# google/neural-light-transport

Measured on AMD Instinct MI355X. Metric: rendered Mtexels/s at 1024^2 UV (full Model.call forward: U-Net + UV->camera warp); at N > 1: N collective-free replicas of this forward (weak scaling).  The data-parallel TRAIN step with the RCCL gradient all-reduce (BASELINE config 4) is `train_step`: value = Mtexels/s over all ranks, speedup_vs_o, higher is better.
Workload: dtype f32 via 3xbf16 split, 9 exact products, fp32 accumulate (the LDS-tiled encoder convs: fp32 operands as three bf16 terms on v_mfma_f32_16x16x32_bf16, every term product exact in fp32); f32 storage everywhere, every other launch native f32; 1 GPU; BASELINE config 3: dragon_specular relight+view-synth, depth0 16/depth 256, 4 frames/GPU, 1024^2 UV, k=4 obs maps, 512^2 camera warp; frames_per_gpu=4, uv=1024, k=4, cam=512, conv_algo=auto, plan=fused ends, launch=eager, two HIP streams, distinct_batches_rotated=3, launch_tape_replays=0, parallelism=dp1 (frames sharded, no forward collective), world=1, dist_world_size=1, device=cuda:0

## Files before the change

include/nlt_hip.h:

```cpp
#ifndef NLT_HIP_H_
#define NLT_HIP_H_

#ifdef __cplusplus
extern "C" {
#endif

typedef enum {
  NLT_OK = 0,
  NLT_ERR_BAD_ARG = -1,
  NLT_ERR_UNSUPPORTED = -2,
  NLT_ERR_LAUNCH = -3
} nlt_status;

typedef enum {
  NLT_CONV1X1 = 0,
  NLT_CONV_K2S2 = 1,
  NLT_CONV_K2S1 = 2,
  NLT_DECONV_K2S2 = 3,
  NLT_DECONV_K2S1 = 4,
  NLT_CONV_K3S1 = 5,
  NLT_CONV_K3S2 = 6,
  NLT_DECONV_K3S1 = 7,
  NLT_DECONV_K3S2 = 8
} nlt_conv_mode;
// ... 351 lines not shown
                          const float* p2, int add_base, float alpha, float* q1, int ldq, float* skip3,
                          float* qtmp2, void* stream);
int nlt_front_ovr_forward_u8(const unsigned char* diffuse_store, const unsigned char* cvis_store,
                             const unsigned char* lvis_store, const int* ids, int n, int h, int w,
                             const float* packed, const float* packed_l2, const float* p1, const float* s0,
                             const float* p2, int add_base, float alpha, float* q1, int ldq, float* skip3,
                             float* qtmp2, void* stream);

int nlt_conv_backward_data(int adj_mode, int tile_hint, int ksplit, float* workspace,
                           const float* dpre, int ldp, int cpre, int n, int h, int w,
                           const float* w_packed, const float* zero_bias, int cout, float* out, int ldo,
                           const float* mask_src, int ldm, float mask_alpha, int accumulate,
                           int split_c, const float* split_y, float* split_d, float split_alpha, int split_partial,
                           void* stream);

long nlt_conv_wino_packed_floats(int mode, int cin, int cout, int tn);
int nlt_pack_conv_wino_weights(int mode, const float* w_keras, int cin, int cout, int tn, float* packed, void* stream);
int nlt_conv_wino_forward(int mode, const float* src, int ld, int cin, int frames, int kobs, int h, int w,
                          const float* packed, const float* bias, int cout, int tn,
                          float* out, int ldo, float* mean_out, int ldm, int act, float alpha, void* stream);
int nlt_pack_conv_wino_weights_adjoint(int adj_mode, const float* w_keras, int cpre, int cout, int tn, int full, int lo,
                                       float* packed, void* stream);
int nlt_conv_wino_backward_data(int adj_mode, const float* dpre, int ldp, int cpre, int n, int h, int w,
                                const float* packed, int cout, int tn, float* out, int ldo,
                                const float* mask_src, int ldm, float mask_alpha, int accumulate, void* stream);

int nlt_conv_c32_supported(int mode, int cin, int cout);
int nlt_conv_c32_forward(int mode, const float* src, int ld, int cin, int frames, int kobs, int h, int w,
                         const float* packed, const float* bias, int cout,
                         float* out, int ldo, float* mean_out, int ldm, int act, float alpha, void* stream);

long nlt_conv_tile_packed_floats(int mode, int cin, int cout, int tn);
int nlt_pack_conv_tile_weights(int mode, const float* w_keras, int cin, int cout, int tn, float* packed, void* stream);
int nlt_conv_tile_forward(int mode, const float* src, int ld, int cin, int frames, int kobs, int h, int w,
                          const float* packed, const float* bias, int cout, int tn,
                          float* out, int ldo, float* mean_out, int ldm, int act, float alpha, void* stream);

int nlt_pack_conv_tile_weights_adjoint(int adj_mode, const float* w_keras, int cpre, int cout, int tn, int full, int lo,
                                       float* packed, void* stream);
int nlt_conv_tile_backward_data(int adj_mode, const float* dpre, int ldp, int cpre, int n, int h, int w,
                                const float* packed, int cout, int tn, float* out, int ldo,
                                const float* mask_src, int ldm, float mask_alpha, int accumulate,
                                int split_c, const float* split_y, float* split_d, float split_alpha, int split_partial,
                                void* stream);

long nlt_conv_tile3_packed_elems(int mode, int cin, int cout, int tn);
int nlt_pack_conv_tile3_weights(int mode, const float* w_keras, int cin, int cout, int tn, unsigned short* packed, void* stream);
int nlt_conv_tile3_forward(int mode, int nprod, const float* src, int ld, int cin, int frames, int kobs, int h, int w,
                           const unsigned short* packed, const float* bias, int cout, int tn,
                           float* out, int ldo, float* mean_out, int ldm, int act, float alpha, void* stream);
int nlt_conv_tile3r_forward(int mode, int nprod, const float* src, int ld, int cin, int frames, int kobs, int h, int w,
                            const unsigned short* packed, const float* bias, int cout, int tn,
                            float* out, int ldo, float* mean_out, int ldm, int act, float alpha, int max_workgroups, void* stream);
long nlt_conv_tile3w_s2_packed_elems(int cin2, int cout2);
int nlt_pack_conv_tile3w_s2_weights(const float* w_keras, int cin2, int cout2, unsigned short* packed, void* stream);
long nlt_conv_tile3w_s2_lds_bytes(int cin, int cout, int cout2);
int nlt_conv_tile3w_s2_forward(int nprod, const float* src, int ld, int cin, int frames, int kobs, int h, int w,
                               const unsigned short* packed, const float* bias, int cout, float* out, int ldo,
                               float* mean_out, int ldm, int act, float alpha,
                               const unsigned short* packed2, const float* bias2, int cout2, float* out2, int ldo2,
                               int act2, float alpha2, int max_workgroups, void* stream);

long nlt_chmix_bf16_packed_elems(int cin, int cout);
int nlt_chmix_bf16_pack(const float* w_keras, int cin, int cout, unsigned short* packed, void* stream);
int nlt_chmix_bf16_forward(const unsigned short* x, long texels, int cin, const unsigned short* packed,
                           const float* bias, int cout, int act, float alpha, unsigned short* out, void* stream);

int nlt_conv_k3_forward(int mode, int algo, const float* x, int n, int h, int w, int cin,
                        const float* w_keras, const float* bias, int cout, float* y,
                        int act, float alpha, void* stream);

int nlt_conv_k3_backward_data(int mode, int algo, const float* dpre, int n, int h, int w, int cin,
                              const float* w_keras, int cout, float* dx, void* stream);

long nlt_conv_k3_wgrad_workspace_floats(int mode, int n, int h, int w, int cin, int cout);
int nlt_conv_k3_backward_weights(int mode, const float* x, int n, int h, int w, int cin,
                                 const float* dpre, int cout, float* dw_keras, float* dbias,
                                 float* workspace, long workspace_floats, void* stream);

#ifdef __cplusplus
}
#endif
#endif
```

neural-light-transport_amd/_capi.py:

```python
import ctypes
import threading
import os

import torch

_HERE = os.path.dirname(os.path.abspath(__file__))
LIB_PATH = os.environ.get('NLT_HIP_LIB') or os.path.join(_HERE, 'libnlt_hip.so')

CONV1X1, CONV_K2S2, CONV_K2S1, DECONV_K2S2, DECONV_K2S1 = range(5)
CONV_K3S1, CONV_K3S2, DECONV_K3S1, DECONV_K3S2 = range(5, 9)
ALGO_AUTO, ALGO_DIRECT, ALGO_MFMA = range(3)

_c_int, _c_long, _c_float, _vp = ctypes.c_int, ctypes.c_long, ctypes.c_float, ctypes.c_void_p
_c_double = ctypes.c_double
MAP_F64, MAP_F32, MAP_F16 = range(3)

SIGNATURES = {
    'nlt_version': (ctypes.c_char_p, []),
    'nlt_status_string': (ctypes.c_char_p, [_c_int]),
    'nlt_packed_weight_floats': (_c_long, [_c_int] * 4),
    'nlt_pack_conv_weights': (_c_int, [_c_int, _vp, _c_int, _c_int, _c_int, _vp, _vp]),
    'nlt_conv_forward': (_c_int, [_c_int, _c_int, _c_int, _vp, _c_int, _c_int, _vp, _c_int, _c_int,
                                  _c_int, _c_int, _c_int, _vp, _vp, _vp, _c_int, _vp, _c_int,
                                  _c_int, _c_float, _vp, _c_int, _c_int, _vp]),
# ... 56 lines not shown
    'nlt_front_packed_floats': (_c_long, []),
    'nlt_front_pack_weights': (_c_int, [_vp] * 15 + [_vp]),
    'nlt_front_forward': (_c_int, [_vp] * 5 + [_c_int] * 4 + [_vp, _c_int, _c_float, _vp, _vp, _vp, _vp]),
    'nlt_front_l2_packed_floats': (_c_long, []),
    'nlt_front_pack_l2_weights': (_c_int, [_vp] * 5 + [_vp]),
    'nlt_front2_forward': (_c_int, [_vp] * 5 + [_c_int] * 4 + [_vp, _vp, _c_int, _c_float, _vp, _vp, _vp, _vp, _vp]),
    'nlt_front4_forward': (_c_int, [_vp] * 5 + [_c_int] * 4 + [_vp, _vp, _c_int, _c_float, _vp, _vp, _vp, _vp, _c_int, _vp]),
    'nlt_front4_forward_u8': (_c_int, [_vp] * 6 + [_c_int] * 4 + [_vp, _vp, _c_int, _c_float, _vp, _vp, _vp, _vp, _c_int, _vp]),
    'nlt_front4_forward_train': (_c_int, [_vp] * 5 + [_c_int] * 4 + [_vp, _vp, _c_int, _c_float] + [_vp] * 7 + [_vp]),
    'nlt_dec_block_forward': (_c_int, [_vp, _c_int, _vp, _c_int, _c_int, _c_int, _c_int, _vp, _vp, _vp, _vp, _c_int, _c_float, _vp, _vp]),
    'nlt_back_forward': (_c_int, [_vp] * 3 + [_c_int] * 3 + [_vp] * 5 + [_c_float, _vp, _vp]),
    'nlt_front_forward_train': (_c_int, [_vp] * 5 + [_c_int] * 4 + [_vp, _c_int, _c_float] + [_vp] * 6),
    'nlt_back_forward_train': (_c_int, [_vp] * 3 + [_c_int] * 3 + [_vp] * 5 + [_c_float] + [_vp] * 4),
    'nlt_front_backward_workspace_floats': (_c_long, [_c_int] * 3),
    'nlt_front_backward': (_c_int, [_vp] * 5 + [_c_int] * 4 + [_vp] * 21),
    'nlt_back_backward_workspace_floats': (_c_long, [_c_int] * 3),
    'nlt_back_backward': (_c_int, [_vp] * 5 + [_c_int] * 3 + [_vp] * 3 + [_c_float] + [_vp] * 10),
    'nlt_conv_splitk_workspace_floats': (_c_long, [_c_int] * 6),
    'nlt_conv_forward_splitk': (_c_int, [_c_int, _c_int, _c_int, _vp, _vp, _c_int, _c_int, _vp, _c_int, _c_int,
                                         _c_int, _c_int, _c_int, _vp, _vp, _c_int, _vp, _c_int, _c_int, _c_float,
                                         _vp, _c_int, _c_int, _vp]),
    'nlt_conv_forward_map': (_c_int, [_c_int, _c_int, _c_int, _vp, _vp, _c_int, _c_int, _vp, _c_int, _c_int,
                                      _c_int, _c_int, _c_int, _vp, _vp, _c_int, _vp, _c_int, _c_int, _c_float,
                                      _vp, _c_int, _vp]),
    'nlt_dec_block_forward_map': (_c_int, [_vp, _vp, _c_int, _c_int, _c_int, _c_int, _vp, _vp, _vp, _c_int, _c_float, _vp, _vp, _vp]),
    'nlt_back_forward_map': (_c_int, [_vp, _vp, _c_int, _vp, _c_int, _c_int, _c_int, _vp, _vp, _vp, _vp, _c_float, _vp, _vp, _vp]),
    'nlt_front_ovr_forward': (_c_int, [_vp] * 3 + [_c_int] * 3 + [_vp] * 5 + [_c_int, _c_float, _vp, _c_int, _vp, _vp, _vp]),
    'nlt_front_ovr_forward_u8': (_c_int, [_vp] * 4 + [_c_int] * 3 + [_vp] * 5 + [_c_int, _c_float, _vp, _c_int, _vp, _vp, _vp]),
    'nlt_conv_backward_data': (_c_int, [_c_int, _c_int, _c_int, _vp, _vp, _c_int, _c_int, _c_int, _c_int, _c_int, _vp, _vp, _c_int,
                                        _vp, _c_int, _vp, _c_int, _c_float, _c_int, _c_int, _vp, _vp, _c_float, _c_int, _vp]),
    'nlt_conv_tile_packed_floats': (_c_long, [_c_int] * 4),
    'nlt_pack_conv_tile_weights': (_c_int, [_c_int, _vp, _c_int, _c_int, _c_int, _vp, _vp]),
    'nlt_conv_tile_forward': (_c_int, [_c_int, _vp, _c_int, _c_int, _c_int, _c_int, _c_int, _c_int, _vp, _vp, _c_int, _c_int,
                                       _vp, _c_int, _vp, _c_int, _c_int, _c_float, _vp]),
    'nlt_pack_conv_tile_weights_adjoint': (_c_int, [_c_int, _vp, _c_int, _c_int, _c_int, _c_int, _c_int, _vp, _vp]),
    'nlt_conv_c32_supported': (_c_int, [_c_int] * 3),
    'nlt_conv_c32_forward': (_c_int, [_c_int, _vp, _c_int, _c_int, _c_int, _c_int, _c_int, _c_int, _vp, _vp, _c_int,
                                      _vp, _c_int, _vp, _c_int, _c_int, _c_float, _vp]),
    'nlt_conv_wino_packed_floats': (_c_long, [_c_int] * 4),
    'nlt_pack_conv_wino_weights': (_c_int, [_c_int, _vp, _c_int, _c_int, _c_int, _vp, _vp]),
    'nlt_conv_wino_forward': (_c_int, [_c_int, _vp, _c_int, _c_int, _c_int, _c_int, _c_int, _c_int, _vp, _vp, _c_int, _c_int,
                                       _vp, _c_int, _vp, _c_int, _c_int, _c_float, _vp]),
    'nlt_pack_conv_wino_weights_adjoint': (_c_int, [_c_int, _vp, _c_int, _c_int, _c_int, _c_int, _c_int, _vp, _vp]),
    'nlt_conv_wino_backward_data': (_c_int, [_c_int, _vp, _c_int, _c_int, _c_int, _c_int, _c_int, _vp, _c_int, _c_int, _vp, _c_int,
                                             _vp, _c_int, _c_float, _c_int, _vp]),
    'nlt_conv_tile_backward_data': (_c_int, [_c_int, _vp, _c_int, _c_int, _c_int, _c_int, _c_int, _vp, _c_int, _c_int, _vp, _c_int,
                                             _vp, _c_int, _c_float, _c_int, _c_int, _vp, _vp, _c_float, _c_int, _vp]),
    'nlt_conv_tile3_packed_elems': (_c_long, [_c_int] * 4),
    'nlt_pack_conv_tile3_weights': (_c_int, [_c_int, _vp, _c_int, _c_int, _c_int, _vp, _vp]),
    'nlt_conv_tile3_forward': (_c_int, [_c_int, _c_int, _vp, _c_int, _c_int, _c_int, _c_int, _c_int, _c_int, _vp, _vp, _c_int, _c_int,
                                        _vp, _c_int, _vp, _c_int, _c_int, _c_float, _vp]),
    'nlt_conv_tile3r_forward': (_c_int, [_c_int, _c_int, _vp, _c_int, _c_int, _c_int, _c_int, _c_int, _c_int, _vp, _vp, _c_int, _c_int,
                                         _vp, _c_int, _vp, _c_int, _c_int, _c_float, _c_int, _vp]),
    'nlt_conv_tile3w_s2_packed_elems': (_c_long, [_c_int] * 2),
    'nlt_pack_conv_tile3w_s2_weights': (_c_int, [_vp, _c_int, _c_int, _vp, _vp]),
    'nlt_conv_tile3w_s2_lds_bytes': (_c_long, [_c_int] * 3),
    'nlt_conv_tile3w_s2_forward': (_c_int, [_c_int, _vp, _c_int, _c_int, _c_int, _c_int, _c_int, _c_int, _vp, _vp, _c_int, _vp, _c_int,
                                            _vp, _c_int, _c_int, _c_float, _vp, _vp, _c_int, _vp, _c_int, _c_int, _c_float, _c_int, _vp]),
    'nlt_conv_bf16_packed_elems': (_c_long, [_c_int] * 4),
    'nlt_conv_bf16_pack': (_c_int, [_c_int, _vp, _c_int, _c_int, _c_int, _vp, _vp]),
    'nlt_conv_bf16_forward': (_c_int, [_c_int, _c_int, _vp, _c_int, _c_int, _c_int, _vp, _c_int, _c_int, _c_int,
                                       _c_int, _c_int, _c_int, _vp, _vp, _c_int, _vp, _c_int, _c_int, _c_int, _c_float, _vp]),
    'nlt_conv_bf16_forward_map': (_c_int, [_c_int, _c_int, _vp, _c_int, _c_int, _c_int, _vp, _c_int, _c_int, _c_int,
                                           _c_int, _c_int, _c_int, _vp, _vp, _c_int, _vp, _c_int, _c_int, _c_int, _c_float,
                                           _vp, _c_int, _vp]),
    'nlt_obs_mean_bf16': (_c_int, [_vp, _c_int, _c_int, _c_long, _c_int, _vp, _c_int, _vp]),
    'nlt_chmix_bf16_packed_elems': (_c_long, [_c_int, _c_int]),
    'nlt_chmix_bf16_pack': (_c_int, [_vp, _c_int, _c_int, _vp, _vp]),
    'nlt_chmix_bf16_forward': (_c_int, [_vp, _c_long, _c_int, _vp, _vp, _c_int, _c_int, _c_float, _vp, _vp]),
    'nlt_cosine_map': (_c_int, [_vp] * 4 + [_c_double] * 3 + [_c_long, _vp, _vp, _vp]),
    'nlt_albedo': (_c_int, [_vp, _c_int, _c_long, _vp, _vp, _vp]),
    'nlt_diffuse_base': (_c_int, [_vp, _vp, _c_int, _c_long, _vp, _vp]),
    'nlt_remap_bilinear_u8': (_c_int, [_vp, _c_int, _c_int, _c_int, _vp, _c_int, _c_int, _c_int, _c_int, _c_int, _vp, _vp]),
    'nlt_remap_bilinear_f32': (_c_int, [_vp, _c_int, _c_int, _c_int, _vp, _c_int, _c_int, _c_int, _c_int, _c_int, _vp, _vp]),
    'nlt_uv_index_map_workspace_bytes': (_c_long, [_c_int, _c_int, _c_long]),
    'nlt_uv_index_map': (_c_int, [_vp, _vp, _c_long, _c_int, _c_int, _c_int, _c_int, _c_double, _vp, _vp, _vp, _vp]),
    'nlt_knn_indices': (_c_int, [_vp, _c_int, _vp, _c_int, _c_int, _vp, _vp]),
    'nlt_psnr_sums': (_c_int, [_vp, _vp, _vp, _c_long, _c_int, _vp, _vp, _vp]),
    'nlt_gather_frames_u8': (_c_int, [_vp, _vp, _c_int, _c_long, _vp, _vp]),
    'nlt_assemble_batch': (_c_int, [_vp] * 6 + [_c_int, _c_int, _c_long, _c_int] + [_vp] * 6 + [_vp]),
    'nlt_warp_backward_det_workspace_bytes': (_c_long, [_c_int] * 5),
    'nlt_warp_backward_det': (_c_int, [_vp, _vp] + [_c_int] * 5 + [_vp, _vp, _c_long, _vp]),
    'nlt_resize_bilinear_backward_gather': (_c_int, [_vp] + [_c_int] * 6 + [_vp, _vp]),
    'nlt_loss_det_workspace_floats': (_c_long, [_c_int]),
    'nlt_l2_loss_forward_det': (_c_int, [_vp, _vp, _c_int, _c_long, _vp, _vp, _c_long, _vp]),
    'nlt_l2_loss_weighted_forward_det': (_c_int, [_vp, _vp, _vp, _c_int, _c_long, _c_int, _vp, _vp, _c_long, _vp]),
    'nlt_l2_train_loss_det': (_c_int, [_vp, _vp, _vp, _c_int, _c_long, _c_float, _vp, _vp, _vp, _vp, _c_long, _vp]),
    'nlt_barron_det_slots_floats': (_c_long, [_c_int] * 3),
    'nlt_barron_loss_det': (_c_int, [_vp, _vp, _c_int, _c_int, _c_int, _vp, _vp, _vp, _vp, _c_long, _vp]),
    'nlt_stem_backward_det_workspace_floats': (_c_long, [_c_int] * 4),
    'nlt_stem_backward_det': (_c_int, [_vp] * 6 + [_c_int] * 5 + [_vp] * 6 + [_vp, _c_long, _vp]),
    'nlt_head_backward_det_workspace_floats': (_c_long, [_c_int] * 5),
    'nlt_head_backward_det': (_c_int, [_vp, _c_int, _c_int, _vp, _c_int, _c_int, _vp, _vp, _c_int, _c_int, _c_int,
                                       _vp, _c_int, _vp, _c_int, _vp, _vp, _vp, _c_long, _vp]),
    'nlt_conv_backward_weights_det_workspace_floats': (_c_long, [_c_int] * 7),
    'nlt_conv_backward_weights_det': (_c_int, [_c_int, _c_int, _vp, _c_int, _c_int, _vp, _c_int, _c_int,
                                               _c_int, _c_int, _c_int, _vp, _c_int, _c_int, _vp, _vp, _vp, _c_long, _vp]),
    'nlt_conv_k3_forward': (_c_int, [_c_int, _c_int, _vp, _c_int, _c_int, _c_int, _c_int, _vp, _vp, _c_int, _vp, _c_int, _c_float, _vp]),
    'nlt_conv_k3_backward_data': (_c_int, [_c_int, _c_int, _vp, _c_int, _c_int, _c_int, _c_int, _vp, _c_int, _vp, _vp]),
    'nlt_conv_k3_wgrad_workspace_floats': (_c_long, [_c_int] * 6),
    'nlt_conv_k3_backward_weights': (_c_int, [_c_int, _vp, _c_int, _c_int, _c_int, _c_int, _vp, _c_int, _vp, _vp, _vp, _c_long, _vp]),
}

_real = None


# ... 808 lines not shown


def pack_conv_wino_weights(mode, w_keras, cin, cout, tn, full=None, lo=0):
    src = (mode, _ptr(_dense(w_keras, 'w_keras')), cin, cout, tn)
    if full is None:
        name, args = 'nlt_pack_conv_wino_weights', src
    else:
        name, args = 'nlt_pack_conv_wino_weights_adjoint', src + (full, lo)
    return _pack('nlt_conv_wino_packed_floats', (mode, cin, cout, tn), name, args, torch.float32, w_keras.device)


def conv_wino_forward(mode, src, ld, cin, frames, kobs, h, w, packed, bias, cout, tn, out, ldo, mean_out, ldm, act=True, alpha=0.3):
    _call('nlt_conv_wino_forward', mode, _ptr(src), ld, cin, frames, kobs, h, w, _ptr(packed), _ptr(bias), cout, tn, _ptr(out), ldo,
          _ptr(mean_out), ldm, 1 if act else 0, float(alpha))


def conv_wino_backward_data(adj_mode, dpre, cpre, ldp, n, h, w, packed, cout, tn, out, ldo, mask_src=None, ldm=0, mask_alpha=0.3,
                            accumulate=False):
    _call('nlt_conv_wino_backward_data', adj_mode, _ptr(dpre), ldp, cpre, n, h, w, _ptr(packed), cout, tn, _ptr(out), ldo,
          _ptr(mask_src), ldm, float(mask_alpha), 1 if accumulate else 0)


def pack_conv_tile3_weights(mode, w_keras, cin, cout, tn):
    return _pack('nlt_conv_tile3_packed_elems', (mode, cin, cout, tn),
                 'nlt_pack_conv_tile3_weights', (mode, _ptr(_dense(w_keras, 'w_keras')), cin, cout, tn), torch.int16, w_keras.device)


def conv_tile3_forward(mode, src, ld, cin, frames, kobs, h, w, packed, bias, cout, tn, out, ldo, mean_out, ldm,
                       act=True, alpha=0.3, nprod=6):
    _call('nlt_conv_tile3_forward', mode, nprod, _ptr(src), ld, cin, frames, kobs, h, w, packed.data_ptr(), _ptr(bias), cout, tn,
          _ptr(out), ldo, _ptr(mean_out), ldm, 1 if act else 0, float(alpha))


def conv_tile3r_plan(mode, cin, tn):
    if mode not in (CONV_K2S1, CONV_K2S2) or cin % 16 or tn not in (32, 64):
        return None
    if mode == CONV_K2S1 and tn == 32:
        for rows in (4, 2):
            lds = cin * 768 + 8 * 6 * (((rows + 1) * 17 + 15) // 16 * 16) * 16
            if lds <= 160 * 1024:
                return (lds, 8, 1, rows)
    lds = cin * (tn // 16) * 384 + 2 * 6 * (160 if mode == CONV_K2S1 else 272) * 16
    if lds > 160 * 1024:
        return None
    return (lds, 8, 1, 8) if 2 * lds > 160 * 1024 else (lds, 4, 2, 8)


def conv_tile3r_forward(mode, src, ld, cin, frames, kobs, h, w, packed, bias, cout, tn, out, ldo, mean_out, ldm,
                        act=True, alpha=0.3, nprod=6, max_workgroups=0):
    _call('nlt_conv_tile3r_forward', mode, nprod, _ptr(src), ld, cin, frames, kobs, h, w, packed.data_ptr(), _ptr(bias), cout, tn,
          _ptr(out), ldo, _ptr(mean_out), ldm, 1 if act else 0, float(alpha), max_workgroups)


def pack_conv_tile3w_s2_weights(w_keras, cin2, cout2):
    return _pack('nlt_conv_tile3w_s2_packed_elems', (cin2, cout2),
                 'nlt_pack_conv_tile3w_s2_weights', (_ptr(_dense(w_keras, 'w_keras')), cin2, cout2), torch.int16, w_keras.device)


def conv_tile3w_s2_plan(cin, cout, cout2):
    n = lib().nlt_conv_tile3w_s2_lds_bytes(cin, cout, cout2)
    return n if n > 0 else None


def conv_tile3w_s2_forward(src, ld, cin, frames, kobs, h, w, packed, bias, cout, mean_out, ldm, packed2, bias2, cout2, out2, ldo2,
                           act=True, alpha=0.3, act2=True, alpha2=0.3, nprod=6, max_workgroups=0, out=None, ldo=0):
    _call('nlt_conv_tile3w_s2_forward', nprod, _ptr(src), ld, cin, frames, kobs, h, w, packed.data_ptr(), _ptr(bias), cout,
          _ptr(out), ldo, _ptr(mean_out), ldm, 1 if act else 0, float(alpha), packed2.data_ptr(), _ptr(bias2), cout2,
          _ptr(out2), ldo2, 1 if act2 else 0, float(alpha2), max_workgroups)


def conv_bf16_pack(mode, w_keras, c0, c1, cout):
    return _pack('nlt_conv_bf16_packed_elems', (mode, c0, c1, cout),
                 'nlt_conv_bf16_pack', (mode, _ptr(_dense(w_keras, 'w_keras')), c0, c1, cout), torch.bfloat16, w_keras.device)


def _any_ptr(t, what):
    if t is None:
        return None, 0
    if not (t.is_cuda and t.dtype in (torch.float32, torch.bfloat16)):
        raise NLTError("%s: expected a float32 / bfloat16 CUDA tensor, got %s on %s" % (what, t.dtype, t.device))
    return t.data_ptr(), 1 if t.dtype == torch.float32 else 0


def conv_bf16_forward(mode, src0, c0, ld0, src1, c1, ld1, n, h, w, w_packed, bias, cout, out, ldo, act=True, alpha=0.3, tile_hint=0):
    p0, f0 = _any_ptr(src0, 'src0')
    p1, f1 = _any_ptr(src1, 'src1')
    po, fo = _any_ptr(out, 'out')
    _call('nlt_conv_bf16_forward', mode, tile_hint, p0, ld0, c0, f0, p1, ld1, c1, f1, n, h, w,
          _tptr(w_packed, torch.bfloat16, 'w_packed'), _ptr(bias), cout, po, ldo, fo, 1 if act else 0, float(alpha))


def conv_bf16_forward_map(mode, src0, c0, ld0, src1, c1, ld1, n, h, w, w_packed, bias, cout, out, ldo, bias_map,
                          act=True, alpha=0.3, tile_hint=0):
    p0, f0 = _any_ptr(src0, 'src0')
    p1, f1 = _any_ptr(src1, 'src1')
    po, fo = _any_ptr(out, 'out')
    _call('nlt_conv_bf16_forward_map', mode, tile_hint, p0, ld0, c0, f0, p1, ld1, c1, f1, n, h, w,
          _tptr(w_packed, torch.bfloat16, 'w_packed'), _ptr(bias), cout, po, ldo, fo, 1 if act else 0, float(alpha),
          _tptr(bias_map, torch.float32, 'bias_map'), bias_map.shape[0])


def obs_mean_bf16(obs, n, k, hw, c, out, ldo):
    if obs.dtype != torch.bfloat16 or out.dtype != torch.bfloat16:
        raise NLTError("obs_mean_bf16: bfloat16 tensors expected")
    _call('nlt_obs_mean_bf16', obs.data_ptr(), n, k, hw, c, out.data_ptr(), ldo)

# ... 252 lines not shown
```

neural-light-transport_amd/csrc/conv_tile3.hip:

```cpp
#include "nlt_common.h"
#include "pack_common.h"

namespace {

typedef __attribute__((ext_vector_type(8))) __bf16 bf16x8;
typedef unsigned short u16;
typedef unsigned int u32x4 __attribute__((ext_vector_type(4)));

constexpr int TH = 8, TW = 16;
constexpr int QS2 = 272, ODD2 = 132;
constexpr int PL = 160;

template <int MODE> struct T3;
template <> struct T3<NLT_CONV_K2S1> { static constexpr int PAIRS = 2, B_UNITS = 153 * 2, B_SLOTS = 6 * PL; };
template <> struct T3<NLT_CONV_K2S2> { static constexpr int PAIRS = 1, B_UNITS = 256 * 2, B_SLOTS = 6 * QS2; };

struct Tile3P {
  const float* src; const u16* packed; const float* bias;
  float* out; float* mean_out;
  int ld, cin, frames, kobs, h, w;
  int oh, ow, cout, ldo, ldm;
  int tiles_y, tiles_x, ncc;
  int act; float alpha;
};
// ... 241 lines not shown
  };
  auto store_b = [&](int buf) {
    u32x4* base = lds + 2 * A_SLOTS + buf * TT::B_SLOTS;
#pragma unroll
    for (int n = 0; n < NB; ++n)
      if (b_st[n]) split_store_unit(base + b_lds[n], BPL, rb[n][0], rb[n][1]);
  };

  f32x4 acc[KO][RT][CT], mean[RT][CT];
#pragma unroll
  for (int rt = 0; rt < RT; ++rt)
#pragma unroll
    for (int ct = 0; ct < CT; ++ct) {
      mean[rt][ct] = (f32x4){0.f, 0.f, 0.f, 0.f};
#pragma unroll
      for (int io = 0; io < KO; ++io) acc[io][rt][ct] = mean[rt][ct];
    }

  load_a(0);
  load_b(0, 0);
  store_a(0);
  store_b(0);
  __syncthreads();
  int q = 0;
  for (int gi = 0; gi < groups; ++gi) {
    for (int s = 0; s < spf; ++s) {
      const int sa = (gi * spf + s) & 1;
#pragma unroll
      for (int io = 0; io < KO; ++io, ++q) {
        const bool more = q + 1 < total;
        const bool new_slab = io + 1 == KO;
        int ns = s, ngi = gi;
        if (new_slab) { if (++ns == spf) { ns = 0; ++ngi; } }
        if (more) {
          if (new_slab) load_a(ns);
          load_b(ns, ngi * KO + (new_slab ? 0 : io + 1));
        }
        stage_products<MODE, TNT, NPROD>(lds + sa * A_SLOTS, lds + 2 * A_SLOTS + (q & 1) * TT::B_SLOTS, lane, wm, wn, acc[io]);
        if (s == spf - 1 && io == KO - 1) {
#pragma unroll
          for (int e = 0; e < KO; ++e)
            epilogue<false>(p, f, gi * KO + e, (g * TNT + wn * CT) * 16 + 4 * kk, ty0 + wm * RT, tx0 + j, acc[e], mean);
        }
        if (more) {
          if (new_slab) store_a(sa ^ 1);
          store_b((q + 1) & 1);
        }
        __syncthreads();
      }
    }
  }
}

extern __shared__ u32x4 tile3r_lds[];

template <int MODE, int TNT, int NPROD, int KO, int NWV>
__global__ __launch_bounds__(64 * NWV, 2) void conv_tile3r_kernel(Tile3P p, int ngroups) {
  using TT = T3<MODE>;
  constexpr int NT = 64 * NWV;
  constexpr int WN = TNT == 4 ? 2 : 1, WM = NWV / WN, RT = TH / WM, CT = 2;
  constexpr int A_SLOTS = TT::PAIRS * TNT * 3 * 64;
  constexpr int NB = (TT::B_UNITS + NT - 1) / NT;
  constexpr int BPL = MODE == NLT_CONV_K2S1 ? PL : QS2;
  const int a_group = p.ncc * 2 * TNT * 3 * 64;
  u32x4* const lds_b = tile3r_lds + a_group;

  const int tid = threadIdx.x, lane = tid & 63, wave = tid >> 6;
  const int kk = lane >> 4, j = lane & 15;
  const int wn = wave % WN, wm = wave / WN;
  const int spf = (MODE == NLT_CONV_K2S1 ? 1 : 2) * p.ncc;
  const int groups = p.kobs / KO;
  const long in_frame = (long)p.h * p.w;
  const int tiles = p.frames * p.tiles_y * p.tiles_x;
  const long items = (long)tiles * ngroups;
  const int rank = xcd_tile3(blockIdx.x, gridDim.x);
  int it = (int)(rank * items / gridDim.x);
  const int it_end = (int)((rank + 1) * items / gridDim.x);
  if (it >= it_end) return;

  int b_lds[NB], b_hf[NB]; long b_tex[NB]; bool b_ok[NB], b_st[NB];
#pragma unroll
  for (int i = 0; i < NB; ++i) unit_slot<MODE>(tid + NT * i, b_hf[i], b_lds[i], b_st[i]);
  int ng = 0, nf = 0, nty0 = 0, ntx0 = 0;
  auto geom = [&](int item) {
    ng = item / tiles;
    int t = item - ng * tiles;
    ntx0 = (t % p.tiles_x) * TW; t /= p.tiles_x;
    nty0 = (t % p.tiles_y) * TH;
    nf = t / p.tiles_y;
#pragma unroll
    for (int i = 0; i < NB; ++i) unit_source<MODE>(p, unit_texel(tid + NT * i), b_st[i], nty0, ntx0, b_ok[i], b_tex[i]);
  };

  f32x4 rb[NB][2];
  auto load_b = [&](int s, int frame) {
    const int cc = MODE == NLT_CONV_K2S1 ? s : (s >> 1);
    const int a = MODE == NLT_CONV_K2S1 ? 0 : (s & 1);
    const float* sp = p.src + ((long)(nf * p.kobs + frame) * in_frame + (long)a * p.w) * p.ld + cc * 16;
#pragma unroll
    for (int n = 0; n < NB; ++n) gather_unit(sp, p.ld, b_ok[n], b_tex[n], b_hf[n], rb[n][0], rb[n][1]);
  };
  auto store_b = [&](int buf) {
    u32x4* base = lds_b + buf * TT::B_SLOTS;
#pragma unroll
    for (int n = 0; n < NB; ++n)
      if (b_st[n]) split_store_unit(base + b_lds[n], BPL, rb[n][0], rb[n][1]);
// ... 461 lines not shown
  return NLT_OK;
}

}

extern "C" long nlt_conv_tile3_packed_elems(int mode, int cin, int cout, int tn) {
  if ((mode != NLT_CONV_K2S1 && mode != NLT_CONV_K2S2) || cin <= 0 || cout <= 0) return -1;
  if ((cin & 15) || (tn != 32 && tn != 64) || cout % tn) return -1;
  return (long)12 * cin * cout;
}

extern "C" int nlt_pack_conv_tile3_weights(int mode, const float* w_keras, int cin, int cout, int tn, unsigned short* packed,
                                           void* stream) {
  const long total = nlt_conv_tile3_packed_elems(mode, cin, cout, tn);
  if (total <= 0) return NLT_ERR_UNSUPPORTED;
  if (!w_keras || !packed || !nlt_aligned16(packed)) return NLT_ERR_BAD_ARG;
  hipLaunchKernelGGL(pack_tile3_kernel, dim3((unsigned)((total + 255) / 256)), dim3(256), 0, static_cast<hipStream_t>(stream),
                     w_keras, cin, cout, tn / 16, total, packed);
  NLT_CHECK_LAUNCH();
  return NLT_OK;
}

static int tile3_forward(int mode, int nprod, const float* src, int ld, int cin, int frames, int kobs, int h, int w,
                         const unsigned short* packed, const float* bias, int cout, int tn,
                         float* out, int ldo, float* mean_out, int ldm, int act, float alpha, int resident_wg, void* stream) {
  const bool own_args = (out || mean_out) && (nprod == 1 || nprod == 3 || nprod == 6 || nprod == 9);
  const bool supported = nlt_conv_tile3_packed_elems(mode, cin, cout, tn) > 0 && !(mode == NLT_CONV_K2S2 && ((h | w) & 1));
  Tile3P p;
  const int st = tile3_params(p, own_args, supported, true, ldo, mode == NLT_CONV_K2S2, src, ld, cin, frames, kobs, h, w, packed, bias,
                              cout, out, ldo, mean_out, ldm, act, alpha);
  if (st != NLT_OK) return st;
  hipStream_t s = static_cast<hipStream_t>(stream);
  if (mode == NLT_CONV_K2S1)
    return tn == 64 ? launch3<NLT_CONV_K2S1, 4>(p, nprod, s, resident_wg) : launch3<NLT_CONV_K2S1, 2>(p, nprod, s, resident_wg);
  return tn == 64 ? launch3<NLT_CONV_K2S2, 4>(p, nprod, s, resident_wg) : launch3<NLT_CONV_K2S2, 2>(p, nprod, s, resident_wg);
}

extern "C" int nlt_conv_tile3_forward(int mode, int nprod, const float* src, int ld, int cin, int frames, int kobs, int h, int w,
                                      const unsigned short* packed, const float* bias, int cout, int tn,
                                      float* out, int ldo, float* mean_out, int ldm, int act, float alpha, void* stream) {
  return tile3_forward(mode, nprod, src, ld, cin, frames, kobs, h, w, packed, bias, cout, tn, out, ldo, mean_out, ldm, act, alpha,
                       -1, stream);
}

extern "C" int nlt_conv_tile3r_forward(int mode, int nprod, const float* src, int ld, int cin, int frames, int kobs, int h, int w,
                                       const unsigned short* packed, const float* bias, int cout, int tn,
                                       float* out, int ldo, float* mean_out, int ldm, int act, float alpha, int max_workgroups,
                                       void* stream) {
  if (max_workgroups < 0) return NLT_ERR_BAD_ARG;
  return tile3_forward(mode, nprod, src, ld, cin, frames, kobs, h, w, packed, bias, cout, tn, out, ldo, mean_out, ldm, act, alpha,
                       max_workgroups, stream);
}

extern "C" long nlt_conv_tile3w_s2_packed_elems(int cin2, int cout2) {
  return (cin2 == 32 && cout2 == 64) ? (long)12 * cin2 * cout2 : -1;
}

extern "C" int nlt_pack_conv_tile3w_s2_weights(const float* w_keras, int cin2, int cout2, unsigned short* packed, void* stream) {
  const long total = nlt_conv_tile3w_s2_packed_elems(cin2, cout2);
  if (total <= 0) return NLT_ERR_UNSUPPORTED;
  if (!w_keras || !packed || !nlt_aligned16(packed)) return NLT_ERR_BAD_ARG;
  hipLaunchKernelGGL(pack_tile3s2_kernel, dim3((unsigned)((total + 255) / 256)), dim3(256), 0, static_cast<hipStream_t>(stream),
                     w_keras, cin2, cout2, total, packed);
  NLT_CHECK_LAUNCH();
  return NLT_OK;
}

extern "C" long nlt_conv_tile3w_s2_lds_bytes(int cin, int cout, int cout2) {
  return (cin == 32 && cout == 32 && cout2 == 64 && S2_LDS <= TILE3R_LDS_CU) ? (long)S2_LDS : -1;
}

extern "C" int nlt_conv_tile3w_s2_forward(int nprod, const float* src, int ld, int cin, int frames, int kobs, int h, int w,
                                          const unsigned short* packed, const float* bias, int cout, float* out, int ldo,
                                          float* mean_out, int ldm, int act, float alpha,
                                          const unsigned short* packed2, const float* bias2, int cout2, float* out2, int ldo2,
                                          int act2, float alpha2, int max_workgroups, void* stream) {
  const bool own_args = packed2 && bias2 && out2 && max_workgroups >= 0 && cout2 > 0;
  const bool supported = nlt_conv_tile3w_s2_lds_bytes(cin, cout, cout2) > 0 && (nprod == 6 || nprod == 9) && !((h | w) & 1) && !out;
  const bool own_layout = ldo2 >= cout2 && !(ldo2 & 3) && nlt_aligned16(packed2) && nlt_aligned16(bias2) && nlt_aligned16(out2);
  Tile3S2P P;
  const int st = tile3_params(P.a, own_args, supported, own_layout, ldo2, false, src, ld, cin, frames, kobs, h, w, packed, bias, cout,
                              out, ldo, mean_out, ldm, act, alpha);
  if (st != NLT_OK) return st;
  P.packed2 = packed2; P.bias2 = bias2; P.out2 = out2; P.ldo2 = ldo2; P.act2 = act2; P.alpha2 = alpha2;
  return launch3w_s2(P, nprod, max_workgroups, static_cast<hipStream_t>(stream));
}
```

neural-light-transport_amd/engine.py:

```python
import os

import torch

from . import _capi as C
from .engine_infer import OverrideMixin


class OpTimer:

    def __init__(self):
        self.pending, self.records = [], {}
        self.flops = {}
        self.moved = {}

    def launch(self, label, nbytes, fn, *args, **kw):
        e0, e1 = torch.cuda.Event(enable_timing=True), torch.cuda.Event(enable_timing=True)
        e0.record()
        fn(*args, **kw)
        e1.record()
        self.pending.append((label, nbytes, e0, e1))

    def collect(self):
        torch.cuda.synchronize()
        for label, nbytes, e0, e1 in self.pending:
            r = self.records.setdefault(label, [0, 0.0, nbytes])
            r[0] += 1
            r[1] += e0.elapsed_time(e1)
        self.pending = []
        return self.records


def _act_kw(act):
    return {'act': act is not None, 'alpha': act.alpha if act is not None else 0.0}


def _gemm(mode, n, h, w, cin, cout):
    ncols = cout * (4 if mode == C.DECONV_K2S2 else 1)
    taps = 4 if mode in (C.CONV_K2S2, C.CONV_K2S1, C.DECONV_K2S1) else 1
    rows = n * h * w // (4 if mode == C.CONV_K2S2 else 1)
    return rows, ncols, 2 * rows * taps * cin * ncols


CHOICE_DICTS = {'tile': ('tile_hints',), 'direct': ('algo_hints',), 'lds': ('lds_hints',), 'splitk': ('tile_hints', 'splitk_hints'),
                'wino': ('wino_hints',), 'c32': ('c32_hints',)}
HINT_DICTS = tuple(dict.fromkeys(a for attrs in CHOICE_DICTS.values() for a in attrs))
EXCLUSIVE = ('lds', 'wino', 'c32')


def hint_word(hint):
    return hint & 255, bool(hint & 256), bool(hint & 512)


FOLD_S2 = 1024
FOLD_HINT = FOLD_S2 + 512 + 32


class RenderPlan(OverrideMixin):
    def __init__(self, net_query, net_obs, use_obs=True):
        self.timer = None
        self.q, self.o, self.use_obs = net_query, net_obs, use_obs
        self.tile_hints = {}
        self.algo_hints = {}
        self.lds_hints = {}
        self.splitk_hints = {}
        self.wino_hints = {}
        self.c32_hints = {}
        self._trial = None
        self._ran = set()
        self.autotune = os.environ.get('NLT_AUTOTUNE', '1') != '0'
        self.fuse_ends = os.environ.get('NLT_FUSED', '1') != '0'
        self._front_blob = None
        self.fuse_override = os.environ.get('NLT_FUSED_OVERRIDE', '1') != '0'
        self._ovr = None
        self.front_l2 = os.environ.get('NLT_FRONT_L2', '1') != '0'
        self.fuse_dec = os.environ.get('NLT_FUSED_DEC', '1') != '0'
        self.front_v4 = os.environ.get('NLT_FRONT4', '1') != '0'
        self.fuse_train = os.environ.get('NLT_FUSED_TRAIN', '1') != '0'
        self.front4_train = os.environ.get('NLT_FRONT4_TRAIN', '1') != '0'
        self.two_streams = os.environ.get('NLT_STREAMS', '2') != '1'
        self._side = None
        self._bside = None
        self.wgrad_tiled = os.environ.get('NLT_WGRAD', 'tiled') != 'atomic'
        self.wgrad_narrow = os.environ.get('NLT_WGRAD_NARROW', '1') != '0'
        self.bwd_streams = int(os.environ.get('NLT_BWD_STREAMS', '1'))
        self.use_tape = os.environ.get('NLT_TAPE', '1') != '0'
        self.fold_split = os.environ.get('NLT_FOLD_SPLIT', '1') != '0'
        self.tile_dgrad = os.environ.get('NLT_TILE_DGRAD', '1') != '0'
        self._tuning = False
        self.tune_backward = os.environ.get('NLT_TUNE_BWD', '1') != '0'
        self.precision = os.environ.get('NLT_PRECISION', 'fp32')
        self._pred_out = None
        self._pred_slot = 'back_infer'
        self.prune_packs = os.environ.get('NLT_PRUNE_PACKS', '1') != '0'
        self.grad_hook = None
        self.grad_mid_level = 0
        self.generation = 0
        self.tape_replays = 0
        self.use_wino = os.environ.get('NLT_WINO', '1') != '0'
        self.use_c32 = os.environ.get('NLT_C32', '1') != '0'
        self.fold_s2 = os.environ.get('NLT_FOLD_S2', '1') != '0'
        self.alias_obs = os.environ.get('NLT_ALIAS_OBS', '1') != '0'
        is_c = net_query.is_contracting
        self.n_down = sum(is_c) - 1
        self.n_up = len(is_c) - sum(is_c) - 1
        assert self.n_down == self.n_up
        self._bufs = {}
# ... 169 lines not shown
        self._launch(label, 4 * (n * h * w * (c0 + c1) + n * oh * ow * layer.n_ch_out), fn, layer.mode,
                     src0, c0, ld0, src1, c1, ld1, n, h, w, layer.packed_bf16(c0, c1), layer.bias.detach(), layer.n_ch_out, out, ldo,
                     *extra, **_act_kw(act), tile_hint=0 if self._trial is not None else self.tile_hints.get('bf.' + label, 0),
                     flops=_gemm(layer.mode, n, h, w, c0 + c1, layer.n_ch_out)[2], moved=moved)

    def _fold_ok(self, layer, cin, nxt):
        return (self.fold_s2 and self.precision in ('f32x3', 'f32x3_9') and layer.kernel.is_cuda and layer.mode == C.CONV_K2S1
                and nxt.mode == C.CONV_K2S2 and C.conv_tile3w_s2_plan(cin, layer.n_ch_out, nxt.n_ch_out) is not None)

    def _conv_fold(self, label, layer, act, src, cin, ld, frames, kobs, h, w, mean_out, ldm, fold):
        label2, nxt, act2, out2, ldo2 = fold
        nxt.build(layer.n_ch_out, src.device)
        nf, c, c2 = frames * kobs, layer.n_ch_out, nxt.n_ch_out
        nbytes = 4 * (nf * h * w * cin + nf * h * w * c) + 4 * frames * h * w * c * (kobs + 1)
        nbytes += 4 * (nf * h * w * c + nf * (h // 2) * (w // 2) * c2)
        moved = 4 * (nf * h * w * cin + (frames * h * w * c if mean_out is not None else 0) + nf * (h // 2) * (w // 2) * c2)
        self._ran.add((label, 'lds'))
        self._launch(label, nbytes, C.conv_tile3w_s2_forward, src, ld, cin, frames, kobs, h, w, layer.packed_tile3(32),
                     layer.bias.detach(), c, mean_out, ldm, nxt.packed_tile3s2(), nxt.bias.detach(), c2, out2, ldo2,
                     act=act is not None, alpha=act.alpha if act is not None else 0.0,
                     act2=act2 is not None, alpha2=act2.alpha if act2 is not None else 0.0,
                     nprod=9 if self.precision == 'f32x3_9' else 6,
                     flops=2 * nf * h * w * 4 * cin * c + 2 * nf * (h // 2) * (w // 2) * 4 * c * c2, moved=moved)

    def _conv_enc(self, label, layer, act, src, cin, ld, frames, kobs, h, w, out, ldo, algo, mean_out=None, ldm=0,
                  obs_weights=None, fold=None):
        layer.build(cin, src.device)
        conv = (label, layer, act, src, cin, ld, frames, kobs, h, w, out, ldo, mean_out, ldm)
        trial = self._trial is not None
        chint = self._hint('c32', label)
        if (chint and self.use_c32 and algo == C.ALGO_AUTO and obs_weights is None and layer.cin == cin and ld % 4 == 0 and ldo % 4 == 0
                and C.conv_c32_supported(layer.mode, cin, layer.n_ch_out) and not (chint == 2 and kobs == 1 and trial)):
            self._enc_launch(C.conv_c32_forward, layer.packed_tile(32), (), 'c32', chint == 2 and kobs > 1, *conv)
            return
        if (algo == C.ALGO_AUTO and layer.mode == C.CONV_K2S1 and self._hint('wino', label) and self._wino(*conv, obs_weights)):
            return
        hint = self._hint('lds', label)
        tn, unfold, resident = hint_word(hint)
        ok = (tn and obs_weights is None and algo == C.ALGO_AUTO and layer.mode in (C.CONV_K2S2, C.CONV_K2S1)
              and layer.cin == cin and cin % 16 == 0 and layer.n_ch_out % tn == 0)
        if hint & FOLD_S2:
            if ok and fold is not None and hint == FOLD_HINT and ((h | w) & 1) == 0 and self._fold_ok(layer, cin, fold[1]):
                if mean_out is None and kobs == 1:
                    mean_out, ldm = out, ldo
                self._conv_fold(label, layer, act, src, cin, ld, frames, kobs, h, w, mean_out, ldm, fold)
                return True
            ok = ok and not trial
        if ok and resident and (self.precision not in ('f32x3', 'f32x3_9') or C.conv_tile3r_plan(layer.mode, cin, tn) is None):
            ok = not trial
            resident = False
        if ok and unfold and kobs == 1:
            ok = not trial
            unfold = False
        if ok and self.precision in ('f32x3', 'f32x3_9'):
            self._enc_launch(C.conv_tile3r_forward if resident else C.conv_tile3_forward, layer.packed_tile3(tn), (tn,),
                             'lds', unfold, *conv, nprod=9 if self.precision == 'f32x3_9' else 6)
        elif ok:
            self._enc_launch(C.conv_tile_forward, layer.packed_tile(tn), (tn,), 'lds', unfold, *conv)
        else:
            self._conv(label, layer, act, src, cin, ld, None, 0, 0, frames * kobs, h, w, out, ldo, algo)
            if mean_out is not None:
                oh, ow = layer.out_hw(h, w)
                self._mean(label, out, obs_weights, frames, kobs, oh * ow, layer.n_ch_out, mean_out, ldm)

    def _dec_block_plain(self, b, j, lab, da, dact_a, db, dact_b, srcs, n, hh, ww, algo, s2_label=None, bmap=None):
        nl = da.n_ch_out
        self._conv(s2_label or lab + '.s2', da, dact_a, *srcs, n, hh, ww, b['dtmp'][j], nl, algo, bmap=bmap)
        self._conv(lab + '.s1', db, dact_b, b['dtmp'][j], nl, nl, None, 0, 0, n, 2 * hh, 2 * ww, b['dec'][j], db.n_ch_out, algo)
        return b['dec'][j], db.n_ch_out

    def _autotune(self, run, backward=False):
        saved_timer = self.timer
        self._tuning = True
        results = {}
        trials = [('tile', 16 * r + c) for r in (1, 2, 4) for c in (1, 2, 4)]
        if not self.fuse_ends and not backward:
            trials.append(('direct', 0))
        if not backward:
            trials += [('lds', 32), ('lds', 64), ('lds', 256 + 32), ('lds', 256 + 64)]
            if self.precision in ('f32x3', 'f32x3_9'):
                trials += [('lds', 512 + 32), ('lds', 512 + 64)]
                if self.fold_s2 and self._fold_trial():
                    trials.append(('lds', FOLD_HINT))
        elif self.tile_dgrad:
            trials += [('lds', 32), ('lds', 64)]
        if self.use_c32 and not backward:
            trials += [('c32', 1), ('c32', 2)]
        if self.use_wino:
            trials += [('wino', 32), ('wino', 64)] + ([('wino', 256 + 32), ('wino', 256 + 64)] if not backward else [])
        mode = os.environ.get('NLT_SPLITK', 'all')
        if mode == 'all' or (mode == 'fwd' and not backward):
            forms = os.environ.get('NLT_SPLITK_FORMS', 'both')
            cand = ((4, 8, 16, 32, 64, 128) if forms != 'two' else ()) + ((-16, -32, -64, -128) if forms == 'both' else ()) + \
                   ((-4, -8, -16, -32, -64, -128) if forms == 'two' else ())
            trials += [('splitk', (16 * r + c, ks)) for (r, c) in ((1, 1), (1, 2), (2, 2), (1, 4)) for ks in cand]
        try:
            for kind, hint in trials:
                self._trial, self._ran = (kind, hint), set()
                self.timer = None
                run()
                self.timer = OpTimer()
                run(); run()
                rec = self.timer.collect()
                for label, r in rec.items():
                    t = r[1] / r[0]
                    if label.endswith('.o.s1') and label.replace('.s1', '.mean') in rec:
                        m = rec[label.replace('.s1', '.mean')]
                        t += m[1] / m[0]
                    if kind == 'tile' or (label, kind) in self._ran:
                        results.setdefault(label, []).append((t, kind, hint))
        finally:
            self._trial, self.timer, self._tuning = None, saved_timer, False
        for label, res in results.items():
            t_fold = [t for t, kind, hint in res if kind == 'lds' and hint == FOLD_HINT]
            label2 = self._fold_partner(label)
            if t_fold and not backward and label2 in results:
                rest = [r for r in res if not (r[1] == 'lds' and r[2] == FOLD_HINT)]
                if rest and min(t_fold) < min(rest)[0] + min(results[label2])[0]:
                    self.set_choice(label, 'lds', FOLD_HINT)
        for label, res in results.items():
            if '.s1' not in label and '.s2' not in label and label != 'L0.q':
                continue
            _, kind, hint = min(r for r in res if not (r[1] == 'lds' and r[2] == FOLD_HINT))
            if backward and 'dgrad' not in label:
                continue
            self.set_choice(label, kind, hint)
        self.tuned = {**getattr(self, 'tuned', {}), **results}
        self._drop_tapes()
        reg = getattr(self.q.layers[0], '_registry', None)
        if reg is not None and self.prune_packs:
            reg.begin_census()

    def _fold_trial(self):
        k = getattr(self.q.layers[0], 'kernel', None)
        return k is not None and k.is_cuda

    @staticmethod
    def _fold_partner(label):
        parts = label.split('.')
        if len(parts) != 3 or parts[1:] != ['o', 's1'] or not parts[0][1:].isdigit():
            return None
        return 'L%d.o.s2' % (int(parts[0][1:]) + 1)

    def _drop_tapes(self):
        for b in self._bufs.values():
            b.pop('tapes', None)

    def export_tuning(self):
        return {a: dict(getattr(self, a)) for a in HINT_DICTS}

    def import_tuning(self, d):
        for a in HINT_DICTS:
            getattr(self, a).update(d.get(a, {}))
        self.autotune = False
        self._drop_tapes()

    def save_tuning(self, path):
        import json
        with open(path, 'w') as f:
            json.dump(self.export_tuning(), f)

    def load_tuning(self, path):
        import json
        with open(path) as f:
            self.import_tuning(json.load(f))

    def can_fuse(self, b, obs_weights, obs_override):
        q, D, U, cl = self.q, self.n_down, self.n_up, b['C']
        if not (self.fuse_ends and self.use_obs and obs_weights is None and obs_override is None and D >= 2 and U >= 2):
            return False
        if b['obs'][0].shape[1] > 14 and not self.front_v4:
            return False
        last = q.layers[D + U].convs()
        prev = q.layers[D + U - 1].convs()
        acts = [a for blk in (q.layers[1], self.o.layers[1], q.layers[D + U]) for _, a in blk.convs()]
        return (cl[0] == 16 and cl[1] == 16 and last[0][0].n_ch_out == 4 and last[1][0].n_ch_out == 4
                and prev[1][0].n_ch_out == 8 and q.layers[-1].n_ch_out == 3
                and all(a is not None for a in acts) and len({a.alpha for a in acts}) == 1)

    def _front_weights(self, dev, l2=True):
        q, o, D, U = self.q, self.o, self.n_down, self.n_up
        q0, o0, head = q.layers[0], o.layers[0], q.layers[-1]
        (qa, _), (qb, _) = q.layers[1].convs()
        (oa, _), (ob, _) = o.layers[1].convs()
        q0.build(5, dev); o0.build(3, dev); qa.build(32, dev); qb.build(16, dev); oa.build(16, dev); ob.build(16, dev)
        head.build(36, dev)
# ... 635 lines not shown
```

Baseline: 3785 Mtexels/s.

## Add direct-gather k2s2 tile3 conv kernel as autotune candidate

Adds a new 3xbf16 MFMA encoder conv kernel for stride-2 2x2 convs. It gathers input pixels straight from global memory into registers instead of staging them, double-buffers only the packed weights in LDS, and processes several observation maps per workgroup. The kernel is exposed through the C API and added to the forward autotune trials under a new DIRECT_S2 hint bit, so it only runs when the tuner measures it as fastest. The aim is to cut LDS traffic and syncs for the input operand, at the cost of uncoalesced strided global loads and higher register pressure.

```diff
diff --git a/include/nlt_hip.h b/include/nlt_hip.h
--- a/include/nlt_hip.h
+++ b/include/nlt_hip.h
@@ -427,6 +427,9 @@
 int nlt_conv_tile3r_forward(int mode, int nprod, const float* src, int ld, int cin, int frames, int kobs, int h, int w,
                             const unsigned short* packed, const float* bias, int cout, int tn,
                             float* out, int ldo, float* mean_out, int ldm, int act, float alpha, int max_workgroups, void* stream);
+int nlt_conv_tile3d_forward(int mode, int nprod, const float* src, int ld, int cin, int frames, int kobs, int h, int w,
+                            const unsigned short* packed, const float* bias, int cout, int tn,
+                            float* out, int ldo, float* mean_out, int ldm, int act, float alpha, void* stream);
 long nlt_conv_tile3w_s2_packed_elems(int cin2, int cout2);
 int nlt_pack_conv_tile3w_s2_weights(const float* w_keras, int cin2, int cout2, unsigned short* packed, void* stream);
 long nlt_conv_tile3w_s2_lds_bytes(int cin, int cout, int cout2);
diff --git a/neural-light-transport_amd/_capi.py b/neural-light-transport_amd/_capi.py
--- a/neural-light-transport_amd/_capi.py
+++ b/neural-light-transport_amd/_capi.py
@@ -132,6 +132,8 @@
                                         _vp, _c_int, _vp, _c_int, _c_int, _c_float, _vp]),
     'nlt_conv_tile3r_forward': (_c_int, [_c_int, _c_int, _vp, _c_int, _c_int, _c_int, _c_int, _c_int, _c_int, _vp, _vp, _c_int, _c_int,
                                          _vp, _c_int, _vp, _c_int, _c_int, _c_float, _c_int, _vp]),
+    'nlt_conv_tile3d_forward': (_c_int, [_c_int, _c_int, _vp, _c_int, _c_int, _c_int, _c_int, _c_int, _c_int, _vp, _vp, _c_int, _c_int,
+                                         _vp, _c_int, _vp, _c_int, _c_int, _c_float, _vp]),
     'nlt_conv_tile3w_s2_packed_elems': (_c_long, [_c_int] * 2),
     'nlt_pack_conv_tile3w_s2_weights': (_c_int, [_vp, _c_int, _c_int, _vp, _vp]),
     'nlt_conv_tile3w_s2_lds_bytes': (_c_long, [_c_int] * 3),
@@ -1046,6 +1048,12 @@
           _ptr(out), ldo, _ptr(mean_out), ldm, 1 if act else 0, float(alpha), max_workgroups)
 
 
+def conv_tile3d_forward(mode, src, ld, cin, frames, kobs, h, w, packed, bias, cout, tn, out, ldo, mean_out, ldm,
+                        act=True, alpha=0.3, nprod=6):
+    _call('nlt_conv_tile3d_forward', mode, nprod, _ptr(src), ld, cin, frames, kobs, h, w, packed.data_ptr(), _ptr(bias), cout, tn,
+          _ptr(out), ldo, _ptr(mean_out), ldm, 1 if act else 0, float(alpha))
+
+
 def pack_conv_tile3w_s2_weights(w_keras, cin2, cout2):
     return _pack('nlt_conv_tile3w_s2_packed_elems', (cin2, cout2),
                  'nlt_pack_conv_tile3w_s2_weights', (_ptr(_dense(w_keras, 'w_keras')), cin2, cout2), torch.int16, w_keras.device)
diff --git a/neural-light-transport_amd/csrc/conv_tile3.hip b/neural-light-transport_amd/csrc/conv_tile3.hip
--- a/neural-light-transport_amd/csrc/conv_tile3.hip
+++ b/neural-light-transport_amd/csrc/conv_tile3.hip
@@ -317,6 +317,130 @@
   }
 }
 
+__device__ __forceinline__ void gather_b_s2(const float* q8, f32x4& v0, f32x4& v1) {
+  v0 = *reinterpret_cast<const f32x4*>(q8);
+  v1 = *reinterpret_cast<const f32x4*>(q8 + 4);
+}
+__device__ __forceinline__ void terms_b_s2(bool ok, const f32x4& v0, const f32x4& v1, bf16x8& hi, bf16x8& mid, bf16x8& lo) {
+  const f32x4 z = {0.f, 0.f, 0.f, 0.f};
+  u32x4 t[3];
+  split8(ok ? v0 : z, ok ? v1 : z, t[0], t[1], t[2]);
+  hi = __builtin_bit_cast(bf16x8, t[0]);
+  mid = __builtin_bit_cast(bf16x8, t[1]);
+  lo = __builtin_bit_cast(bf16x8, t[2]);
+}
+
+template <int TNT, int NPROD, int KO>
+__global__ __launch_bounds__(256, TNT * KO >= 8 ? 2 : 3) void conv_tile3d_kernel(Tile3P p) {
+  constexpr int WM = 4, RT = TH / WM, CT = TNT;
+  constexpr int A_SLOTS = TNT * 3 * 64;
+  constexpr int NA = (A_SLOTS + 255) / 256;
+  constexpr int NM = 2 * KO;
+  __shared__ u32x4 lds[2 * A_SLOTS];
+  p.mean_out = nullptr;
+
+  const int tid = threadIdx.x, lane = tid & 63, wm = tid >> 6;
+  const int kk = lane >> 4, j = lane & 15;
+  int tile = xcd_tile3(blockIdx.x, gridDim.x);
+  const int tx0 = (tile % p.tiles_x) * TW; tile /= p.tiles_x;
+  const int ty0 = (tile % p.tiles_y) * TH;
+  const int f = tile / p.tiles_y;
+  const int g = blockIdx.y;
+  const int groups = p.kobs / KO;
+  const int nouter = groups * p.ncc;
+  const long in_frame = (long)p.h * p.w;
+
+  int b_off[RT]; bool b_ok[RT];
+#pragma unroll
+  for (int rt = 0; rt < RT; ++rt) {
+    const int y = ty0 + wm * RT + rt, x = tx0 + j;
+    b_ok[rt] = y < p.oh && x < p.ow;
+    b_off[rt] = (b_ok[rt] ? (2 * y * p.w + 2 * x + (kk >> 1)) * p.ld : 0) + 8 * (kk & 1);
+  }
+
+  u32x4 ra[NA];
+  f32x4 rb[2][RT][2];
+  auto load_a = [&](int cc, int a) {
+    const u32x4* ap = reinterpret_cast<const u32x4*>(p.packed) + (((long)g * p.ncc + cc) * 2 + a) * A_SLOTS;
+#pragma unroll
+    for (int n = 0; n < NA; ++n) ra[n] = ap[(A_SLOTS % 256 == 0 || tid + 256 * n < A_SLOTS) ? tid + 256 * n : tid];
+  };
+  auto store_a = [&](int buf) {
+    u32x4* base = lds + buf * A_SLOTS;
+#pragma unroll
+    for (int n = 0; n < NA; ++n)
+      if (A_SLOTS % 256 == 0 || tid + 256 * n < A_SLOTS) base[tid + 256 * n] = ra[n];
+  };
+  auto load_b = [&](int u, int gi, int cc, int a, int io) {
+    const float* sp = p.src + ((long)(f * p.kobs + gi * KO + io) * in_frame + (long)a * p.w) * p.ld + cc * 16;
+#pragma unroll
+    for (int rt = 0; rt < RT; ++rt) gather_b_s2(sp + b_off[rt], rb[u][rt][0], rb[u][rt][1]);
+  };
+
+  f32x4 acc[KO][RT][CT], mean[RT][CT];
+#pragma unroll
+  for (int rt = 0; rt < RT; ++rt)
+#pragma unroll
+    for (int ct = 0; ct < CT; ++ct) {
+      mean[rt][ct] = (f32x4){0.f, 0.f, 0.f, 0.f};
+#pragma unroll
+      for (int io = 0; io < KO; ++io) acc[io][rt][ct] = mean[rt][ct];
+    }
+
+  load_a(0, 0);
+  load_b(0, 0, 0, 0, 0);
+  load_b(1, 0, 0, 1 / KO, 1 % KO);
+  store_a(0);
+  __syncthreads();
+  int gi = 0, cc = 0;
+  for (int o = 0; o < nouter; ++o) {
+    int ngi = gi, nc = cc + 1;
+    if (nc == p.ncc) { nc = 0; ++ngi; }
+    if (o + 1 == nouter) { ngi = gi; nc = cc; }
+#pragma unroll
+    for (int m = 0; m < NM; ++m) {
+      const int a = m / KO, io = m % KO, u = m & 1;
+      bf16x8 bt[3][RT], at[3][CT];
+#pragma unroll
+      for (int rt = 0; rt < RT; ++rt) terms_b_s2(b_ok[rt], rb[u][rt][0], rb[u][rt][1], bt[0][rt], bt[1][rt], bt[2][rt]);
+      if (io == 0) {
+        if (a == 0) load_a(cc, 1);
+        else load_a(nc, 0);
+      }
+      if (m + 2 < NM) load_b(u, gi, cc, (m + 2) / KO, (m + 2) % KO);
+      else load_b(u, ngi, nc, (m + 2 - NM) / KO, (m + 2 - NM) % KO);
+      __builtin_amdgcn_sched_barrier(0);
+      read_a(lds + a * A_SLOTS, 0, lane, at);
+      term_products<NPROD>(at, [&](int t, int rt) { return bt[t][rt]; }, acc[io]);
+      if (m == NM - 1 && cc == p.ncc - 1) {
+#pragma unroll
+        for (int e = 0; e < KO; ++e) epilogue<false>(p, f, gi * KO + e, g * TNT * 16 + 4 * kk, ty0 + wm * RT, tx0 + j, acc[e], mean);
+      }
+      if (io == KO - 1) {
+        store_a(a ^ 1);
+        __syncthreads();
+      }
+    }
+    gi = ngi; cc = nc;
+  }
+}
+
+template <int TNT, int KO>
+int launch3d_k(const Tile3P& p, int nprod, hipStream_t s) {
+  const dim3 grid((unsigned)((long)p.frames * p.tiles_y * p.tiles_x), (unsigned)(p.cout / (16 * TNT)));
+  if (nprod == 9) hipLaunchKernelGGL((conv_tile3d_kernel<TNT, 9, KO>), grid, dim3(256), 0, s, p);
+  else hipLaunchKernelGGL((conv_tile3d_kernel<TNT, 6, KO>), grid, dim3(256), 0, s, p);
+  NLT_CHECK_LAUNCH();
+  return NLT_OK;
+}
+
+template <int TNT>
+int launch3d(const Tile3P& p, int nprod, hipStream_t s) {
+  if (TNT == 2 && p.kobs % 4 == 0) return launch3d_k<TNT, (TNT == 2 ? 4 : 1)>(p, nprod, s);
+  if (p.kobs % 2 == 0) return launch3d_k<TNT, 2>(p, nprod, s);
+  return launch3d_k<TNT, 1>(p, nprod, s);
+}
+
 extern __shared__ u32x4 tile3r_lds[];
 
 template <int MODE, int TNT, int NPROD, int KO, int NWV>
@@ -884,6 +1008,19 @@
                        max_workgroups, stream);
 }
 
+extern "C" int nlt_conv_tile3d_forward(int mode, int nprod, const float* src, int ld, int cin, int frames, int kobs, int h, int w,
+                                       const unsigned short* packed, const float* bias, int cout, int tn,
+                                       float* out, int ldo, float* mean_out, int ldm, int act, float alpha, void* stream) {
+  const bool supported = mode == NLT_CONV_K2S2 && nlt_conv_tile3_packed_elems(mode, cin, cout, tn) > 0 && !((h | w) & 1) &&
+                         (nprod == 6 || nprod == 9) && !mean_out;
+  Tile3P p;
+  const int st = tile3_params(p, out != nullptr, supported, true, ldo, true, src, ld, cin, frames, kobs, h, w, packed, bias, cout,
+                              out, ldo, mean_out, ldm, act, alpha);
+  if (st != NLT_OK) return st;
+  hipStream_t s = static_cast<hipStream_t>(stream);
+  return tn == 64 ? launch3d<4>(p, nprod, s) : launch3d<2>(p, nprod, s);
+}
+
 extern "C" long nlt_conv_tile3w_s2_packed_elems(int cin2, int cout2) {
   return (cin2 == 32 && cout2 == 64) ? (long)12 * cin2 * cout2 : -1;
 }
diff --git a/neural-light-transport_amd/engine.py b/neural-light-transport_amd/engine.py
--- a/neural-light-transport_amd/engine.py
+++ b/neural-light-transport_amd/engine.py
@@ -52,6 +52,7 @@
 
 
 FOLD_S2 = 1024
+DIRECT_S2 = 2048
 FOLD_HINT = FOLD_S2 + 512 + 32
 
 
@@ -327,9 +328,14 @@
         if ok and unfold and kobs == 1:
             ok = not trial
             unfold = False
+        direct = bool(hint & DIRECT_S2)
+        if ok and direct and not (self.precision in ('f32x3', 'f32x3_9') and layer.mode == C.CONV_K2S2 and ((h | w) & 1) == 0
+                                  and (mean_out is None or unfold)):
+            ok = not trial
+            direct = False
         if ok and self.precision in ('f32x3', 'f32x3_9'):
-            self._enc_launch(C.conv_tile3r_forward if resident else C.conv_tile3_forward, layer.packed_tile3(tn), (tn,),
-                             'lds', unfold, *conv, nprod=9 if self.precision == 'f32x3_9' else 6)
+            fn = C.conv_tile3d_forward if direct else (C.conv_tile3r_forward if resident else C.conv_tile3_forward)
+            self._enc_launch(fn, layer.packed_tile3(tn), (tn,), 'lds', unfold, *conv, nprod=9 if self.precision == 'f32x3_9' else 6)
         elif ok:
             self._enc_launch(C.conv_tile_forward, layer.packed_tile(tn), (tn,), 'lds', unfold, *conv)
         else:
@@ -355,6 +361,8 @@
             trials += [('lds', 32), ('lds', 64), ('lds', 256 + 32), ('lds', 256 + 64)]
             if self.precision in ('f32x3', 'f32x3_9'):
                 trials += [('lds', 512 + 32), ('lds', 512 + 64)]
+                if self._direct_trial():
+                    trials += [('lds', DIRECT_S2 + u + tn) for u in (0, 256) for tn in (32, 64)]
                 if self.fold_s2 and self._fold_trial():
                     trials.append(('lds', FOLD_HINT))
         elif self.tile_dgrad:
@@ -407,6 +415,10 @@
             reg.begin_census()
 
     def _fold_trial(self):
+        k = getattr(self.q.layers[0], 'kernel', None)
+        return k is not None and k.is_cuda
+
+    def _direct_trial(self):
         k = getattr(self.q.layers[0], 'kernel', None)
         return k is not None and k.is_cuda
 
```

Measured after the change: 3869 Mtexels/s, median of 6. 1.02x the previous value.
